# kallenordling/cesm_emulator

Measured on AMD Instinct MI355X. Metric: train samples/sec (192x288xT frames), higher is better.
Workload: dtype bf16; 1 GPU; config/more_blocks train step, F=12, 192x288, per-GPU batch 8; global_batch=8, frames=12, parallelism=dp1

## Files before the change

### cesm_emulator_amd/csrc/conv_wgrad.hip

```cpp
#include "conv_common.h"

namespace {

constexpr int WG_BP = 32;

template <typename T>
__global__ __launch_bounds__(256) void conv_wgrad_kernel(const T* __restrict__ x1, const T* __restrict__ x2,
                                                         const T* __restrict__ dy1, const T* __restrict__ dy2,
                                                         float* __restrict__ slab, ConvGeom g, int64_t M,
                                                         int64_t px_per_split) {
  constexpr int VEC = sizeof(T) == 2 ? 8 : 4;
  constexpr int ROW = 64;
  constexpr int LDR = sizeof(T) == 2 ? 64 : 65;
  __shared__ __attribute__((aligned(16))) T tY[2][WG_BP * LDR];
  __shared__ __attribute__((aligned(16))) T tX[2][WG_BP * LDR];

  const int tid = threadIdx.x, lane = tid & 63, wid = tid >> 6;
  const int wr = wid >> 1, wc = wid & 1;
  const int Cin = g.C1 + g.C2;
  const int co0 = blockIdx.x * 64;
  const int kcol0 = blockIdx.y * 64;
  const int tap = kcol0 / Cin;
  const int ci0 = kcol0 - tap * Cin;
  const int ky = tap / g.KW, kx = tap - ky * g.KW;
// ... 264 lines not shown
    for (int j = 0; j < 4; ++j) {
#pragma unroll
      for (int half = 0; half < 2; ++half) {
        const int r = lg * 8 + half * 4 + q;
        const int ch = ((j * 16 >> 2) + pp) ^ wgb_swz<64>(r);
        const s16x4 v = __builtin_amdgcn_ds_read_tr16_b64_v4i16((LDS_PTR(s16x4))(tX[buf] + r * 64 + ch * 4));
#pragma unroll
        for (int e = 0; e < 4; ++e) bfr[j][half * 4 + e] = __builtin_bit_cast(bf16, (short)v[e]);
      }
    }
#pragma unroll
    for (int i = 0; i < MT; ++i)
#pragma unroll
      for (int j = 0; j < 4; ++j) acc[i][j] = __builtin_amdgcn_mfma_f32_16x16x32_bf16(af[i], bfr[j], acc[i][j], 0, 0, 0);
    if constexpr (BIAS) {
      if (bias_blk) {
#pragma unroll
        for (int i = 0; i < MT; ++i) bacc[i] = __builtin_amdgcn_mfma_f32_16x16x32_bf16(af[i], ones, bacc[i], 0, 0, 0);
      }
    }
    if (s + 1 < nsteps) sstore(std::integral_constant<int, buf ^ 1>{});
    __syncthreads();
  };
  for (int s = 0; s < nsteps; s += 2) {
    step(s, I0{});
    if (s + 1 < nsteps) step(s + 1, I1{});
  }
  if (BIAS && bias_blk && lr == 0) {
#pragma unroll
    for (int i = 0; i < (BIAS ? MT : 1); ++i)
#pragma unroll
      for (int r = 0; r < 4; ++r) bslab[(int64_t)bz * g.Cout + co0 + wid * (BM / 4) + i * 16 + lg * 4 + r] = bacc[i][r];
  }
  const int K = g.KH * g.KW * Cin;
  float* out = slab + (int64_t)bz * g.Cout * K;
#pragma unroll
  for (int i = 0; i < MT; ++i)
#pragma unroll
    for (int j = 0; j < 4; ++j) {
      const int kc = kcol0 + j * 16 + lr;
#pragma unroll
      for (int r = 0; r < 4; ++r) {
        const int co = co0 + wid * (BM / 4) + i * 16 + lg * 4 + r;
        out[(int64_t)co * K + kc] = acc[i][j][r];
      }
    }
}

template <int BM, int BN, bool BIAS = false>
__global__ __launch_bounds__(512) __attribute__((amdgpu_waves_per_eu(2))) void wgrad_sq_kernel(
    const bf16* __restrict__ x, const bf16* __restrict__ dy, float* __restrict__ slab, float* __restrict__ bslab, int M,
    int Cout, int Cin, int px_per_split) {
  constexpr int WR = BM / 64, WC = 8 / WR, MT = 4, NT = BN / (16 * WC);
  static_assert((BM == 256 || BM == 64) && NT >= 1, "wgrad_sq tiles");
  constexpr int TY = WG_BP * BM / 8, TX = WG_BP * BN / 8;
  constexpr int NY = (TY + 511) / 512, NX = (TX + 511) / 512;
  __shared__ __attribute__((aligned(16))) bf16 tY[2][WG_BP * BM];
  __shared__ __attribute__((aligned(16))) bf16 tX[2][WG_BP * BN];
  const int tid = threadIdx.x, lane = tid & 63, wid = tid >> 6;
  const int lr = lane & 15, lg = lane >> 4;
  const int wr = wid % WR, wc = wid / WR;
  const int co0 = blockIdx.x * BM, k0 = blockIdx.y * BN;
  const int pbeg = blockIdx.z * px_per_split;
  const int pend = min(M, pbeg + px_per_split);
  bf16x8 yr2[2][NY], xr2[2][NX];
  auto gload = [&](int p0, auto slotc) {
    constexpr int slot = decltype(slotc)::value;
#pragma unroll
    for (int u = 0; u < NY; ++u) {
      const int v = tid + 512 * u, r = v / (BM / 8), c = (v % (BM / 8)) * 8;
      const int m = p0 + r;
      yr2[slot][u] = m < pend && v < TY ? *reinterpret_cast<const bf16x8*>(dy + (int64_t)m * Cout + co0 + c) : bf16x8{};
    }
#pragma unroll
    for (int u = 0; u < NX; ++u) {
      const int v = tid + 512 * u, r = v / (BN / 8), c = (v % (BN / 8)) * 8;
      const int m = p0 + r;
      xr2[slot][u] = m < pend && v < TX ? *reinterpret_cast<const bf16x8*>(x + (int64_t)m * Cin + k0 + c) : bf16x8{};
    }
  };
  auto sstore = [&](auto bufc) {
    constexpr int buf = decltype(bufc)::value;
#pragma unroll
    for (int u = 0; u < NY; ++u) {
      const int v = tid + 512 * u, r = v / (BM / 8), c = (v % (BM / 8)) * 8;
      if (v < TY) *reinterpret_cast<bf16x8*>(tY[buf] + r * BM + (((c >> 2) ^ wgb_swz<BM>(r)) * 4)) = yr2[buf][u];
    }
#pragma unroll
    for (int u = 0; u < NX; ++u) {
      const int v = tid + 512 * u, r = v / (BN / 8), c = (v % (BN / 8)) * 8;
      if (v < TX) *reinterpret_cast<bf16x8*>(tX[buf] + r * BN + (((c >> 2) ^ wgb_swz<BN>(r)) * 4)) = xr2[buf][u];
    }
  };
  f32x4 acc[MT][NT];
#pragma unroll
  for (int i = 0; i < MT; ++i)
#pragma unroll
    for (int j = 0; j < NT; ++j) acc[i][j] = f32x4{0.f, 0.f, 0.f, 0.f};
  const bool bias_w = BIAS && blockIdx.y == 0 && wc == 0;
  f32x4 bacc[BIAS ? MT : 1];
#pragma unroll
  for (int i = 0; i < (BIAS ? MT : 1); ++i) bacc[i] = f32x4{0.f, 0.f, 0.f, 0.f};
  bf16x8 ones;
#pragma unroll
  for (int e = 0; e < 8; ++e) ones[e] = (bf16)1.f;
  const int nsteps = (pend - pbeg + WG_BP - 1) / WG_BP;
  using I0 = std::integral_constant<int, 0>;
  using I1 = std::integral_constant<int, 1>;
  if (nsteps > 0) {
    gload(pbeg, I0{});
    if (nsteps > 1) gload(pbeg + WG_BP, I1{});
    sstore(I0{});
  }
  __syncthreads();
  const int q = lr >> 2, pp = lr & 3;
  auto step = [&](int s, auto bufc) {
    constexpr int buf = decltype(bufc)::value;
    if (s + 2 < nsteps) gload(pbeg + (s + 2) * WG_BP, bufc);
    bf16x8 af[MT], bfr[NT];
#pragma unroll
    for (int i = 0; i < MT; ++i) {
      const int c0 = wr * 64 + i * 16;
#pragma unroll
      for (int half = 0; half < 2; ++half) {
        const int r = lg * 8 + half * 4 + q;
        const int ch = ((c0 >> 2) + pp) ^ wgb_swz<BM>(r);
        const s16x4 v = __builtin_amdgcn_ds_read_tr16_b64_v4i16((LDS_PTR(s16x4))(tY[buf] + r * BM + ch * 4));
#pragma unroll
        for (int e = 0; e < 4; ++e) af[i][half * 4 + e] = __builtin_bit_cast(bf16, (short)v[e]);
      }
    }
#pragma unroll
    for (int j = 0; j < NT; ++j) {
      const int c0 = wc * (BN / WC) + j * 16;
#pragma unroll
      for (int half = 0; half < 2; ++half) {
        const int r = lg * 8 + half * 4 + q;
        const int ch = ((c0 >> 2) + pp) ^ wgb_swz<BN>(r);
        const s16x4 v = __builtin_amdgcn_ds_read_tr16_b64_v4i16((LDS_PTR(s16x4))(tX[buf] + r * BN + ch * 4));
#pragma unroll
        for (int e = 0; e < 4; ++e) bfr[j][half * 4 + e] = __builtin_bit_cast(bf16, (short)v[e]);
      }
    }
#pragma unroll
    for (int i = 0; i < MT; ++i)
#pragma unroll
      for (int j = 0; j < NT; ++j) acc[i][j] = __builtin_amdgcn_mfma_f32_16x16x32_bf16(af[i], bfr[j], acc[i][j], 0, 0, 0);
    if constexpr (BIAS) {
      if (bias_w) {
#pragma unroll
        for (int i = 0; i < MT; ++i) bacc[i] = __builtin_amdgcn_mfma_f32_16x16x32_bf16(af[i], ones, bacc[i], 0, 0, 0);
      }
    }
    if (s + 1 < nsteps) sstore(std::integral_constant<int, buf ^ 1>{});
    __syncthreads();
  };
  for (int s = 0; s < nsteps; s += 2) {
    step(s, I0{});
    if (s + 1 < nsteps) step(s + 1, I1{});
  }
  if (BIAS && bias_w && lr == 0) {
#pragma unroll
    for (int i = 0; i < (BIAS ? MT : 1); ++i)
#pragma unroll
      for (int r = 0; r < 4; ++r) bslab[(int64_t)blockIdx.z * Cout + co0 + wr * 64 + i * 16 + lg * 4 + r] = bacc[i][r];
  }
  float* out = slab + (int64_t)blockIdx.z * Cout * Cin;
#pragma unroll
  for (int i = 0; i < MT; ++i)
#pragma unroll
    for (int j = 0; j < NT; ++j) {
      const int kc = k0 + wc * (BN / WC) + j * 16 + lr;
#pragma unroll
      for (int r = 0; r < 4; ++r) {
        const int co = co0 + wr * 64 + i * 16 + lg * 4 + r;
        out[(int64_t)co * Cin + kc] = acc[i][j][r];
      }
    }
}

constexpr int W3_TH = 8, W3_TW = 32;
constexpr int W3_HW = W3_TW + 2, W3_NPIX = (W3_TH + 2) * (W3_TW + 2);
constexpr int W3_P = 48;

__device__ __forceinline__ int w3_swz_dy(int r) { return (((r >> 1) & 1) << 2) | (((r >> 3) & 1) << 3); }
__device__ __forceinline__ int w3_swz_x(int r) { return ((r >> 3) & 1) << 2; }

constexpr int W3_PLANE = (W3_TH + 2) * W3_P * 32;

constexpr int WG_NT = 512;
constexpr int WG_NI = 2;
__global__ __launch_bounds__(WG_NT, 1) void wgrad3x3c64_kernel(const bf16* __restrict__ x1, const bf16* __restrict__ x2,
                                                             const bf16* __restrict__ dy1, const bf16* __restrict__ dy2,
                                                             float* __restrict__ slab, ConvGeom g, int tiles_x,
                                                             int ntiles) {
  __shared__ __attribute__((aligned(16))) bf16 sdy[W3_TH * W3_TW * 64];
  __shared__ __attribute__((aligned(16))) bf16 shx[2 * W3_PLANE];
  const int tid = threadIdx.x, lane = tid & 63, wid = tid >> 6;
  const int cot0 = (wid >> 2) * 2, cit = wid & 3;
  const int co0 = blockIdx.x * 64, ci0 = blockIdx.y * 64;
  const int Cin = g.C1 + g.C2;
  const bf16* xs; int xcs, xcc;
  if (ci0 < g.C1) { xs = x1; xcs = g.C1; xcc = ci0; } else { xs = x2; xcs = g.C2; xcc = ci0 - g.C1; }
  const bf16* ys; int ycs, ycc;
  const int Co2 = g.Cout - g.Co1;
  if (co0 < g.Co1) { ys = dy1; ycs = g.Co1; ycc = co0; } else { ys = dy2; ycs = Co2; ycc = co0 - g.Co1; }
  const int tiles_per_img = tiles_x * ((g.Ho + W3_TH - 1) / W3_TH);

  f32x4 acc[WG_NI][9];
#pragma unroll
  for (int i = 0; i < WG_NI; ++i)
#pragma unroll
    for (int t = 0; t < 9; ++t) acc[i][t] = f32x4{0.f, 0.f, 0.f, 0.f};

  const int lr = lane & 15, lg = lane >> 4, q = lr >> 2, pp = lr & 3;
  const bf16* shp = shx + (cit >> 1) * W3_PLANE;
  int aoff[WG_NI][2], boff[2][3];
#pragma unroll
  for (int half = 0; half < 2; ++half) {
    const int r = lg * 8 + half * 4 + q;
#pragma unroll
    for (int i = 0; i < WG_NI; ++i) aoff[i][half] = r * 64 + ((((cot0 + i) * 4 + pp) ^ w3_swz_dy(r)) * 4);
#pragma unroll
    for (int kx = 0; kx < 3; ++kx) boff[half][kx] = (r + kx) * 32 + ((((cit & 1) * 4 + pp) ^ w3_swz_x(r + kx)) * 4);
  }
  constexpr int YV = 2048 / WG_NT, HV = (W3_NPIX * 8 + WG_NT - 1) / WG_NT;
  bf16x8 yv[YV], hv[HV];
  auto gload = [&](int tile) {
    const int n = tile / tiles_per_img;
    const int rem = tile - n * tiles_per_img;
    const int ty = rem / tiles_x, tx = rem - ty * tiles_x;
    const int y0 = ty * W3_TH, x0 = tx * W3_TW;
#pragma unroll
    for (int k = 0; k < YV; ++k) {
      const int e = tid + k * WG_NT;
      const int p = e >> 3, part = e & 7;
      const int oy = y0 + (p >> 5), ox = x0 + (p & 31);
      const bool ok = oy < g.Ho && ox < g.Wo;
      const bf16x8 v = *reinterpret_cast<const bf16x8*>(
          ys + (ok ? (((int64_t)n * g.Ho + oy) * g.Wo + ox) * ycs : 0) + ycc + part * 8);
      yv[k] = ok ? v : bf16x8{};
    }
#pragma unroll
    for (int k = 0; k < HV; ++k) {
      const int e = tid + k * WG_NT;
      const int hp = e >> 3, part = e & 7;
      const int r = hp / W3_HW, c = hp - r * W3_HW;
      const int iy = y0 - 1 + r, ix = x0 - 1 + c;
      const bool ok = e < W3_NPIX * 8 && (unsigned)iy < (unsigned)g.Hi && (unsigned)ix < (unsigned)g.Wi;
      const bf16x8 v = *reinterpret_cast<const bf16x8*>(
          xs + (ok ? (((int64_t)n * g.Hi + iy) * g.Wi + ix) * xcs : 0) + xcc + part * 8);
      hv[k] = ok ? v : bf16x8{};
    }
  };
  __shared__ __attribute__((aligned(16))) int tdump[WG_NT];
  auto touch = [&](int tile) {
    const int n = tile / tiles_per_img;
    const int rem = tile - n * tiles_per_img;
    const int ty = rem / tiles_x, tx = rem - ty * tiles_x;
    const int y0 = ty * W3_TH, x0 = tx * W3_TW;
    const int64_t yimg = (int64_t)g.Ho * g.Wo * ycs, ximg = (int64_t)g.Hi * g.Wi * xcs;
    const __amdgpu_buffer_rsrc_t yrs =
        __builtin_amdgcn_make_buffer_rsrc((void*)(ys + n * yimg + ycc), (short)0, (int)(yimg * 2 - ycc * 2), 0x00020000);
    const __amdgpu_buffer_rsrc_t xrs =
        __builtin_amdgcn_make_buffer_rsrc((void*)(xs + n * ximg + xcc), (short)0, (int)(ximg * 2 - xcc * 2), 0x00020000);
    auto* dst = (__attribute__((address_space(3))) void*)(tdump + wid * 64);
    {
      const int p = tid & 255;
      const int oy = y0 + (p >> 5), ox = x0 + (p & 31);
      const bool ok = tid < 256 && oy < g.Ho && ox < g.Wo;
      __builtin_amdgcn_raw_ptr_buffer_load_lds(yrs, dst, 4, ok ? (oy * g.Wo + ox) * ycs * 2 : 0x7ffffff0, 0, 0, 0);
    }
    {
      const int hp = tid < 256 ? 256 + tid : tid - 256;
      const int r = hp / W3_HW, c = hp - r * W3_HW;
      const int iy = y0 - 1 + r, ix = x0 - 1 + c;
      const bool ok = hp < W3_NPIX && (unsigned)iy < (unsigned)g.Hi && (unsigned)ix < (unsigned)g.Wi;
      __builtin_amdgcn_raw_ptr_buffer_load_lds(xrs, dst, 4, ok ? (iy * g.Wi + ix) * xcs * 2 : 0x7ffffff0, 0, 0, 0);
    }
  };
  if ((int)blockIdx.z < ntiles) gload(blockIdx.z);
  for (int tile = blockIdx.z; tile < ntiles; tile += gridDim.z) {
    __syncthreads();
#pragma unroll
    for (int k = 0; k < YV; ++k) {
      const int e = tid + k * WG_NT;
      const int p = e >> 3, part = e & 7;
      const int ch = (part * 2) ^ w3_swz_dy(p);
      *reinterpret_cast<bf16x8*>(sdy + p * 64 + ch * 4) = yv[k];
    }
#pragma unroll
    for (int k = 0; k < HV; ++k) {
      const int e = tid + k * WG_NT;
      if (e < W3_NPIX * 8) {
        const int hp = e >> 3, part = e & 7;
        const int r = hp / W3_HW, row = r * W3_P + (hp - r * W3_HW);
        const int ch = ((part & 3) * 2) ^ w3_swz_x(row);
        *reinterpret_cast<bf16x8*>(shx + (part >> 2) * W3_PLANE + row * 32 + ch * 4) = hv[k];
      }
    }
    __syncthreads();
    if (tile + (int)gridDim.z < ntiles) gload(tile + gridDim.z);
    if (tile + 2 * (int)gridDim.z < ntiles) touch(tile + 2 * gridDim.z);
    bf16x8 fa[2][WG_NI], fb[2][9];
    auto rd = [&](int py, int b) {
#pragma unroll
      for (int i = 0; i < WG_NI; ++i)
#pragma unroll
        for (int half = 0; half < 2; ++half) {
          const s16x4 v = __builtin_amdgcn_ds_read_tr16_b64_v4i16((LDS_PTR(s16x4))(sdy + aoff[i][half] + py * 32 * 64));
#pragma unroll
          for (int e = 0; e < 4; ++e) fa[b][i][half * 4 + e] = __builtin_bit_cast(bf16, (short)v[e]);
        }
#pragma unroll
      for (int tap = 0; tap < 9; ++tap) {
        const int ky = tap / 3, kx = tap - ky * 3;
#pragma unroll
        for (int half = 0; half < 2; ++half) {
          const s16x4 v = __builtin_amdgcn_ds_read_tr16_b64_v4i16(
              (LDS_PTR(s16x4))(shp + boff[half][kx] + (py + ky) * W3_P * 32));
#pragma unroll
          for (int e = 0; e < 4; ++e) fb[b][tap][half * 4 + e] = __builtin_bit_cast(bf16, (short)v[e]);
        }
      }
    };
    auto mm = [&](int b) {
#pragma unroll
      for (int tap = 0; tap < 9; ++tap)
#pragma unroll
        for (int i = 0; i < WG_NI; ++i)
          acc[i][tap] = __builtin_amdgcn_mfma_f32_16x16x32_bf16(fa[b][i], fb[b][tap], acc[i][tap], 0, 0, 0);
    };
    rd(0, 0);
#pragma unroll
    for (int py = 0; py < W3_TH; ++py) {
      const int b = py & 1;
      __builtin_amdgcn_sched_barrier(0);
      if (py + 1 < W3_TH) rd(py + 1, b ^ 1);
      mm(b);
      if (py + 1 < W3_TH) {
        constexpr int NRD = 2 * WG_NI + 18, NMF = 9 * WG_NI;
        constexpr int NPAIR = NRD < NMF ? NRD : NMF;
#pragma unroll
        for (int q2 = 0; q2 < NPAIR; ++q2) {
          __builtin_amdgcn_sched_group_barrier(0x100, 1, 0);
          __builtin_amdgcn_sched_group_barrier(0x008, 1, 0);
        }
        if (NRD > NPAIR) __builtin_amdgcn_sched_group_barrier(0x100, NRD - NPAIR, 0);
        if (NMF > NPAIR) __builtin_amdgcn_sched_group_barrier(0x008, NMF - NPAIR, 0);
      }
      __builtin_amdgcn_sched_barrier(0);
    }
  }
  const int K = 9 * Cin;
  float* out = slab + (int64_t)blockIdx.z * g.Cout * K;
#pragma unroll
  for (int i = 0; i < WG_NI; ++i)
#pragma unroll
    for (int tap = 0; tap < 9; ++tap) {
      const int ci = ci0 + cit * 16 + lr;
#pragma unroll
      for (int r = 0; r < 4; ++r) {
        const int co = co0 + (cot0 + i) * 16 + lg * 4 + r;
        out[(int64_t)co * K + tap * Cin + ci] = acc[i][tap][r];
      }
    }
}

template <int BY, int BX>
__device__ __forceinline__ void ws2_taps(const bf16* sdy, const bf16* shx, const int (&aoff)[2][2],
                                         const int (&boff)[2][3], f32x4 (&acc)[2][4]) {
#pragma unroll 1
  for (int py = 0; py < W3_TH; ++py) {
    bf16x8 af[2];
#pragma unroll
    for (int i = 0; i < 2; ++i) {
#pragma unroll
      for (int half = 0; half < 2; ++half) {
        const s16x4 v = __builtin_amdgcn_ds_read_tr16_b64_v4i16((LDS_PTR(s16x4))(sdy + aoff[i][half] + py * 32 * 64));
#pragma unroll
        for (int e = 0; e < 4; ++e) af[i][half * 4 + e] = __builtin_bit_cast(bf16, (short)v[e]);
      }
    }
#pragma unroll
    for (int t = 0; t < 4; ++t) {
      const int oy = BY + (t >> 1), ox = BX + (t & 1);
      bf16x8 bfr;
#pragma unroll
      for (int half = 0; half < 2; ++half) {
        const s16x4 v =
            __builtin_amdgcn_ds_read_tr16_b64_v4i16((LDS_PTR(s16x4))(shx + boff[half][ox] + (py + oy) * W3_P * 32));
#pragma unroll
        for (int e = 0; e < 4; ++e) bfr[half * 4 + e] = __builtin_bit_cast(bf16, (short)v[e]);
      }
      acc[0][t] = __builtin_amdgcn_mfma_f32_16x16x32_bf16(af[0], bfr, acc[0][t], 0, 0, 0);
      acc[1][t] = __builtin_amdgcn_mfma_f32_16x16x32_bf16(af[1], bfr, acc[1][t], 0, 0, 0);
    }
  }
}

__global__ __launch_bounds__(256, 2) void wgrads2_bf16_kernel(const bf16* __restrict__ x, const bf16* __restrict__ dy,
                                                              float* __restrict__ slab, ConvGeom g, int tiles_x,
                                                              int ntiles) {
  __shared__ __attribute__((aligned(16))) bf16 sdy[W3_TH * W3_TW * 64];
  __shared__ __attribute__((aligned(16))) bf16 shx[(W3_TH + 2) * W3_P * 32];
  const int tid = threadIdx.x, lane = tid & 63, wid = tid >> 6;
  const int cot0 = (wid >> 1) * 2, cit = wid & 1;
  const int co0 = blockIdx.x * 64;
  const int ab = (int)blockIdx.y & 3, a = ab >> 1, b = ab & 1;
  const int ci0 = ((int)blockIdx.y >> 2) * 32;
  const int Cin = g.C1;
  const int tiles_per_img = tiles_x * ((g.Ho + W3_TH - 1) / W3_TH);

  f32x4 acc[2][4];
#pragma unroll
  for (int i = 0; i < 2; ++i)
#pragma unroll
    for (int t = 0; t < 4; ++t) acc[i][t] = f32x4{0.f, 0.f, 0.f, 0.f};

  const int lr = lane & 15, lg = lane >> 4, q = lr >> 2, pp = lr & 3;
  int aoff[2][2], boff[2][3];
#pragma unroll
  for (int half = 0; half < 2; ++half) {
    const int r = lg * 8 + half * 4 + q;
#pragma unroll
    for (int i = 0; i < 2; ++i) aoff[i][half] = r * 64 + ((((cot0 + i) * 4 + pp) ^ w3_swz_dy(r)) * 4);
#pragma unroll
    for (int kx = 0; kx < 3; ++kx) boff[half][kx] = (r + kx) * 32 + (((cit * 4 + pp) ^ w3_swz_x(r + kx)) * 4);
  }
  for (int tile = blockIdx.z; tile < ntiles; tile += gridDim.z) {
    const int n = tile / tiles_per_img;
    const int rem = tile - n * tiles_per_img;
    const int ty = rem / tiles_x, tx = rem - ty * tiles_x;
    const int y0 = ty * W3_TH, x0 = tx * W3_TW;
    __syncthreads();
    {
      bf16x8 yv[8], hv[6];
#pragma unroll
      for (int k = 0; k < 8; ++k) {
        const int e = tid + k * 256;
        const int p = e >> 3, part = e & 7;
        const int oy = y0 + (p >> 5), ox = x0 + (p & 31);
        bf16x8 v = {};
        if (oy < g.Ho && ox < g.Wo)
          v = *reinterpret_cast<const bf16x8*>(dy + (((int64_t)n * g.Ho + oy) * g.Wo + ox) * g.Cout + co0 + part * 8);
        yv[k] = v;
      }
#pragma unroll
      for (int k = 0; k < 6; ++k) {
        const int e = tid + k * 256;
        bf16x8 v = {};
        if (e < W3_NPIX * 4) {
          const int hp = e >> 2, part = e & 3;
          const int r = hp / W3_HW, c = hp - r * W3_HW;
          const int iy = 2 * (y0 - 1 + r) + a, ix = 2 * (x0 - 1 + c) + b;
          if ((unsigned)iy < (unsigned)g.Hi && (unsigned)ix < (unsigned)g.Wi)
            v = *reinterpret_cast<const bf16x8*>(x + (((int64_t)n * g.Hi + iy) * g.Wi + ix) * Cin + ci0 + part * 8);
        }
        hv[k] = v;
      }
#pragma unroll
      for (int k = 0; k < 8; ++k) {
        const int e = tid + k * 256;
        const int p = e >> 3, part = e & 7;
        const int ch = (part * 2) ^ w3_swz_dy(p);
        *reinterpret_cast<bf16x8*>(sdy + p * 64 + ch * 4) = yv[k];
      }
#pragma unroll
      for (int k = 0; k < 6; ++k) {
        const int e = tid + k * 256;
        if (e < W3_NPIX * 4) {
          const int hp = e >> 2, part = e & 3;
          const int r = hp / W3_HW, row = r * W3_P + (hp - r * W3_HW);
          const int ch = (part * 2) ^ w3_swz_x(row);
          *reinterpret_cast<bf16x8*>(shx + row * 32 + ch * 4) = hv[k];
        }
      }
    }
    __syncthreads();
    switch (ab) {
      case 0: ws2_taps<1, 1>(sdy, shx, aoff, boff, acc); break;
      case 1: ws2_taps<1, 0>(sdy, shx, aoff, boff, acc); break;
      case 2: ws2_taps<0, 1>(sdy, shx, aoff, boff, acc); break;
      default: ws2_taps<0, 0>(sdy, shx, aoff, boff, acc); break;
    }
  }
  const int K = 16 * Cin;
  float* out = slab + (int64_t)blockIdx.z * g.Cout * K;
#pragma unroll
  for (int i = 0; i < 2; ++i)
#pragma unroll
    for (int t = 0; t < 4; ++t) {
      const int tap = (1 - a + 2 * (t >> 1)) * 4 + (1 - b + 2 * (t & 1));
      const int ci = ci0 + cit * 16 + lr;
#pragma unroll
      for (int r = 0; r < 4; ++r) {
        const int co = co0 + (cot0 + i) * 16 + lg * 4 + r;
        out[(int64_t)co * K + tap * Cin + ci] = acc[i][t][r];
      }
    }
}

constexpr int W36_TH = 8, W36_TW = 36, W36_HW = W36_TW + 2, W36_NPIX = (W36_TH + 2) * W36_HW;
constexpr int W36_NP = W36_TH * W36_TW;

__global__ __launch_bounds__(WG_NT, 1) void wgrad3x3w36c64_kernel(const bf16* __restrict__ x1, const bf16* __restrict__ x2,
                                                                const bf16* __restrict__ dy1, const bf16* __restrict__ dy2,
                                                                float* __restrict__ slab, ConvGeom g, int tiles_x,
                                                                int ntiles) {
  __shared__ __attribute__((aligned(16))) bf16 sdy[W36_NP * 64];
  __shared__ __attribute__((aligned(16))) bf16 shx[2 * W3_PLANE];
  const int tid = threadIdx.x, lane = tid & 63, wid = tid >> 6;
  const int cot0 = (wid >> 2) * 2, cit = wid & 3;
  const int co0 = blockIdx.x * 64, ci0 = blockIdx.y * 64;
  const int Cin = g.C1 + g.C2;
  const bf16* xs; int xcs, xcc;
  if (ci0 < g.C1) { xs = x1; xcs = g.C1; xcc = ci0; } else { xs = x2; xcs = g.C2; xcc = ci0 - g.C1; }
  const bf16* ys; int ycs, ycc;
  const int Co2 = g.Cout - g.Co1;
  if (co0 < g.Co1) { ys = dy1; ycs = g.Co1; ycc = co0; } else { ys = dy2; ycs = Co2; ycc = co0 - g.Co1; }
  const int tiles_per_img = tiles_x * ((g.Ho + W36_TH - 1) / W36_TH);

  f32x4 acc[WG_NI][9];
#pragma unroll
  for (int i = 0; i < WG_NI; ++i)
#pragma unroll
    for (int t = 0; t < 9; ++t) acc[i][t] = f32x4{0.f, 0.f, 0.f, 0.f};

  const int lr = lane & 15, lg = lane >> 4, q = lr >> 2, pp = lr & 3;
  const bf16* shp = shx + (cit >> 1) * W3_PLANE;
  const int cx = (cit & 1) * 4 + pp;
  int aoff[WG_NI][2];
#pragma unroll
  for (int half = 0; half < 2; ++half) {
    const int r = lg * 8 + half * 4 + q;
#pragma unroll
    for (int i = 0; i < WG_NI; ++i) aoff[i][half] = r * 64 + ((((cot0 + i) * 4 + pp) ^ w3_swz_dy(r)) * 4);
  }
  constexpr int YV = (W36_NP * 8 + WG_NT - 1) / WG_NT, HV = (W36_NPIX * 8 + WG_NT - 1) / WG_NT;
  bf16x8 yv[YV], hv[HV];
  auto gload = [&](int tile) {
    const int n = tile / tiles_per_img;
    const int rem = tile - n * tiles_per_img;
    const int ty = rem / tiles_x, tx = rem - ty * tiles_x;
    const int y0 = ty * W36_TH, x0 = tx * W36_TW;
#pragma unroll
    for (int k = 0; k < YV; ++k) {
      const int e = tid + k * WG_NT;
      const int p = e >> 3, part = e & 7;
      const int oy = y0 + p / W36_TW, ox = x0 + (p - (p / W36_TW) * W36_TW);
      const bool ok = e < W36_NP * 8 && oy < g.Ho && ox < g.Wo;
      const bf16x8 v = *reinterpret_cast<const bf16x8*>(
          ys + (ok ? (((int64_t)n * g.Ho + oy) * g.Wo + ox) * ycs : 0) + ycc + part * 8);
      yv[k] = ok ? v : bf16x8{};
    }
#pragma unroll
    for (int k = 0; k < HV; ++k) {
      const int e = tid + k * WG_NT;
      const int hp = e >> 3, part = e & 7;
      const int r = hp / W36_HW, c = hp - r * W36_HW;
      const int iy = y0 - 1 + r, ix = x0 - 1 + c;
      const bool ok = e < W36_NPIX * 8 && (unsigned)iy < (unsigned)g.Hi && (unsigned)ix < (unsigned)g.Wi;
      const bf16x8 v = *reinterpret_cast<const bf16x8*>(
          xs + (ok ? (((int64_t)n * g.Hi + iy) * g.Wi + ix) * xcs : 0) + xcc + part * 8);
      hv[k] = ok ? v : bf16x8{};
    }
  };
  if ((int)blockIdx.z < ntiles) gload(blockIdx.z);
  for (int tile = blockIdx.z; tile < ntiles; tile += gridDim.z) {
    __syncthreads();
#pragma unroll
    for (int k = 0; k < YV; ++k) {
      const int e = tid + k * WG_NT;
      if (e < W36_NP * 8) {
        const int p = e >> 3, part = e & 7;
        const int ch = (part * 2) ^ w3_swz_dy(p);
        *reinterpret_cast<bf16x8*>(sdy + p * 64 + ch * 4) = yv[k];
      }
    }
#pragma unroll
    for (int k = 0; k < HV; ++k) {
      const int e = tid + k * WG_NT;
      if (e < W36_NPIX * 8) {
        const int hp = e >> 3, part = e & 7;
        const int r = hp / W36_HW, row = r * W3_P + (hp - r * W36_HW);
        const int ch = ((part & 3) * 2) ^ w3_swz_x(row);
        *reinterpret_cast<bf16x8*>(shx + (part >> 2) * W3_PLANE + row * 32 + ch * 4) = hv[k];
      }
    }
    __syncthreads();
    if (tile + (int)gridDim.z < ntiles) gload(tile + gridDim.z);
    int prow[2], pcol[2];
#pragma unroll
    for (int half = 0; half < 2; ++half) { prow[half] = 0; pcol[half] = lg * 8 + half * 4 + q; }
    bf16x8 fa[2][WG_NI], fb[2][9];
    auto rd = [&](int kc, int b) {
#pragma unroll
      for (int i = 0; i < WG_NI; ++i)
#pragma unroll
        for (int half = 0; half < 2; ++half) {
          const s16x4 v = __builtin_amdgcn_ds_read_tr16_b64_v4i16((LDS_PTR(s16x4))(sdy + aoff[i][half] + kc * 32 * 64));
#pragma unroll
          for (int e = 0; e < 4; ++e) fa[b][i][half * 4 + e] = __builtin_bit_cast(bf16, (short)v[e]);
        }
      int bo[2][3];
#pragma unroll
      for (int half = 0; half < 2; ++half) {
        const int hb = prow[half] * W3_P + pcol[half];
#pragma unroll
        for (int kx = 0; kx < 3; ++kx) bo[half][kx] = (hb + kx) * 32 + ((cx ^ w3_swz_x(hb + kx)) * 4);
        pcol[half] += 32;
        if (pcol[half] >= W36_TW) { pcol[half] -= W36_TW; ++prow[half]; }
      }
#pragma unroll
      for (int tap = 0; tap < 9; ++tap) {
        const int ky = tap / 3, kx = tap - ky * 3;
#pragma unroll
        for (int half = 0; half < 2; ++half) {
          const s16x4 v = __builtin_amdgcn_ds_read_tr16_b64_v4i16((LDS_PTR(s16x4))(shp + bo[half][kx] + ky * W3_P * 32));
#pragma unroll
          for (int e = 0; e < 4; ++e) fb[b][tap][half * 4 + e] = __builtin_bit_cast(bf16, (short)v[e]);
        }
      }
    };
    auto mm = [&](int b) {
#pragma unroll
      for (int tap = 0; tap < 9; ++tap) {
#pragma unroll
        for (int i = 0; i < WG_NI; ++i)
          acc[i][tap] = __builtin_amdgcn_mfma_f32_16x16x32_bf16(fa[b][i], fb[b][tap], acc[i][tap], 0, 0, 0);
      }
    };
    constexpr int NKC = W36_NP / 32;
    rd(0, 0);
#pragma unroll
    for (int kc = 0; kc < NKC; ++kc) {
      const int b = kc & 1;
      __builtin_amdgcn_sched_barrier(0);
      if (kc + 1 < NKC) rd(kc + 1, b ^ 1);
      mm(b);
      if (kc + 1 < NKC) {
        constexpr int NRD = 2 * WG_NI + 18, NMF = 9 * WG_NI;
        constexpr int NPAIR = NRD < NMF ? NRD : NMF;
#pragma unroll
        for (int q2 = 0; q2 < NPAIR; ++q2) {
          __builtin_amdgcn_sched_group_barrier(0x100, 1, 0);
          __builtin_amdgcn_sched_group_barrier(0x008, 1, 0);
        }
        if (NRD > NPAIR) __builtin_amdgcn_sched_group_barrier(0x100, NRD - NPAIR, 0);
        if (NMF > NPAIR) __builtin_amdgcn_sched_group_barrier(0x008, NMF - NPAIR, 0);
      }
      __builtin_amdgcn_sched_barrier(0);
    }
  }
  const int K = 9 * Cin;
  float* out = slab + (int64_t)blockIdx.z * g.Cout * K;
#pragma unroll
  for (int i = 0; i < WG_NI; ++i)
#pragma unroll
    for (int tap = 0; tap < 9; ++tap) {
      const int ci = ci0 + cit * 16 + lr;
#pragma unroll
      for (int r = 0; r < 4; ++r) {
        const int co = co0 + (cot0 + i) * 16 + lg * 4 + r;
        out[(int64_t)co * K + tap * Cin + ci] = acc[i][tap][r];
      }
    }
}

__global__ __launch_bounds__(256) void conv_wgrad_reduce_kernel(const float* __restrict__ slab, float* __restrict__ dst,
                                                                int nsplit, int Cout, int Cin, int KH, int KW, int swap,
                                                                int flip, int accumulate) {
  const int64_t K = (int64_t)KH * KW * Cin;
  const int64_t total = (int64_t)Cout * K;
  const int64_t e = blockIdx.x * 64ll + (threadIdx.x & 63);
  const int grp = threadIdx.x >> 6;
  float s = 0.f;
  if (e < total) {
    int k = grp;
    for (; k + 28 < nsplit; k += 32) {
      float v[8];
#pragma unroll
      for (int u = 0; u < 8; ++u) v[u] = slab[(int64_t)(k + 4 * u) * total + e];
#pragma unroll
      for (int u = 0; u < 8; ++u) s += v[u];
    }
    for (; k < nsplit; k += 4) s += slab[(int64_t)k * total + e];
  }
  __shared__ float red[4][64];
  red[grp][threadIdx.x & 63] = s;
  __syncthreads();
  if (grp != 0 || e >= total) return;
  s = ((red[0][threadIdx.x] + red[1][threadIdx.x]) + red[2][threadIdx.x]) + red[3][threadIdx.x];
  const int co = (int)(e / K);
  const int kc = (int)(e - (int64_t)co * K);
  const int tap = kc / Cin, ci = kc - tap * Cin;
  int ky = tap / KW, kx = tap - ky * KW;
  if (flip) { ky = KH - 1 - ky; kx = KW - 1 - kx; }
  const int d0 = swap ? ci : co, d1 = swap ? co : ci, D1 = swap ? Cout : Cin;
  const int64_t di = (((int64_t)d0 * D1 + d1) * KH + ky) * KW + kx;
  dst[di] = accumulate ? dst[di] + s : s;
}

template <typename T>
__global__ void colsum_partial_kernel(const T* __restrict__ x, float* __restrict__ part, int64_t rows, int C,
                                      int64_t rows_per_split) {
  const int cq = C / 4;
  const int rl = 256 / cq;
  const int tid = threadIdx.x;
  const int q = tid % cq, rr = tid / cq;
  __shared__ float red[256 * 4];
  float s[4] = {0.f, 0.f, 0.f, 0.f};
  const int64_t r0 = blockIdx.x * rows_per_split;
  const int64_t r1 = min(rows, r0 + rows_per_split);
  if (rr < rl) {
    for (int64_t r = r0 + rr; r < r1; r += rl) {
      float v[4];
      load4(x + r * C + q * 4, v);
      s[0] += v[0]; s[1] += v[1]; s[2] += v[2]; s[3] += v[3];
    }
  }
  for (int i = 0; i < 4; ++i) red[tid * 4 + i] = s[i];
  __syncthreads();
  if (tid < cq) {
    float t[4] = {0.f, 0.f, 0.f, 0.f};
    for (int k = 0; k < rl; ++k)
      for (int i = 0; i < 4; ++i) t[i] += red[(k * cq + tid) * 4 + i];
    for (int i = 0; i < 4; ++i) part[(int64_t)blockIdx.x * C + tid * 4 + i] = t[i];
  }
}

__global__ void colsum_final_kernel(const float* __restrict__ part, float* __restrict__ dst, int nsplit, int C,
                                    int accumulate) {
  const int c = blockIdx.x;
  float s = 0.f;
  for (int k = threadIdx.x; k < nsplit; k += 64) s += part[(int64_t)k * C + c];
  s = wave_sum(s);
  if (threadIdx.x == 0) dst[c] = accumulate ? dst[c] + s : s;
}

enum WgradVariant { WGV_WIDE = 0, WGV_SQ, WGV_GEN, WGV_S2, WGV_W32C64, WGV_W36C64 };

constexpr int WG_BLOCKS = 1024;
constexpr int WG_BLOCKS_BIG = 512;
constexpr int WG_BLOCKS_SQ = 256;
constexpr int WG_BLOCKS_SQ64 = 512;
constexpr int WG_SPLIT_PX = 256;

struct WgradPlan {
  WgradVariant v = WGV_GEN;
  int bm = 64, bn = 64;
  int nsplit = 1;
  bool bias = false;
  bool can_bias = false;
};

static WgradPlan wgrad_plan(int dtype, int Nb, int Hi, int Wi, int C1, int C2, int Ho, int Wo, int Cout, int Co1,
                            int KH, int KW, int S, int P, int U, bool with_bias) {
  WgradPlan pl;
  const bool bf = dtype == CESM_DT_BF16;
  const int Cin = C1 + C2, K = KH * KW * Cin;
  const int64_t M = (int64_t)Nb * Ho * Wo;
  const bool same_hw = Ho == Hi && Wo == Wi, single = C2 == 0 && Co1 == Cout;
  int64_t blocks = WG_BLOCKS, tiles;
  if (bf && KH == 3 && KW == 3 && S == 1 && P == 1 && U == 1 && same_hw) {
    pl.v = ((Wo % W36_TW) == 0 && 5 * Wo <= 4 * (int)cdiv(Wo, W3_TW) * W3_TW) ? WGV_W36C64 : WGV_W32C64;
    blocks = WG_BLOCKS_BIG;
    tiles = (int64_t)(Cout / 64) * (Cin / 32);
  } else if (bf && KH == 4 && KW == 4 && S == 2 && P == 1 && U == 1 && Hi == 2 * Ho && Wi == 2 * Wo && Wo >= 64 &&
             single && !with_bias) {
    pl.v = WGV_S2;
    blocks = WG_BLOCKS_BIG;
    tiles = (int64_t)(Cout / 64) * (Cin / 32) * 4;
  } else {
    const bool wide = bf && M < (1ll << 31);
    int sq = 0;
    if (wide && KH == 1 && KW == 1 && S == 1 && P == 0 && U == 1 && same_hw && single) {
      if (Cout == 64) sq = C1 % 256 == 0 ? 256 : 0;
      else if (Cout % 256 == 0) sq = C1 % 256 == 0 ? 256 : (C1 % 128 == 0 ? 128 : 0);
    }
    pl.v = sq ? WGV_SQ : (wide ? WGV_WIDE : WGV_GEN);
    if (sq) {
      pl.bm = Cout == 64 ? 64 : 256;
      pl.bn = sq;
      blocks = pl.bm == 64 ? WG_BLOCKS_SQ64 : WG_BLOCKS_SQ;
    } else {
      pl.bm = !bf ? 64 : (Cout % 256 == 0 && Co1 % 256 == 0) ? 256 : (Cout % 128 == 0 && Co1 % 128 == 0) ? 128 : 64;
      blocks = pl.bm == 256 ? WG_BLOCKS_BIG : WG_BLOCKS;
    }
    tiles = (int64_t)std::max(1, Cout / pl.bm) * std::max(1, K / pl.bn);
    pl.bias = with_bias && wide;
    pl.can_bias = wide && Co1 == Cout;
  }
  pl.nsplit = (int)std::max<int64_t>(
      1, std::min(blocks / std::max<int64_t>(1, tiles), std::max<int64_t>(1, M / WG_SPLIT_PX)));
  return pl;
}
}

extern "C" {

const char* cesm_conv_wgrad_variant(int dtype, int Nb, int Hi, int Wi, int C1, int C2, int Ho, int Wo, int Cout,
                                    int Co1, int KH, int KW, int S, int P, int U, int with_bias) {
  const WgradPlan pl = wgrad_plan(dtype, Nb, Hi, Wi, C1, C2, Ho, Wo, Cout, Co1, KH, KW, S, P, U, with_bias != 0);
  switch (pl.v) {
    case WGV_W32C64: return "wgrad3x3c64_kernel";
    case WGV_W36C64: return "wgrad3x3w36c64_kernel";
    case WGV_S2: return "wgrads2_bf16_kernel";
    case WGV_SQ: {
      static const char* const sqn[6] = {"wgrad_sq_kernel<64,256>", "wgrad_sq_kernel<64,256,true>",
                                         "wgrad_sq_kernel<256,256>", "wgrad_sq_kernel<256,256,true>",
                                         "wgrad_sq_kernel<256,128>", "wgrad_sq_kernel<256,128,true>"};
      return sqn[(pl.bm == 64 ? 0 : pl.bn == 256 ? 2 : 4) + (with_bias ? 1 : 0)];
    }
    case WGV_WIDE: {
      static const char* const names[6] = {"wgrad_wide_kernel<64,false>", "wgrad_wide_kernel<64,true>",
                                           "wgrad_wide_kernel<128,false>", "wgrad_wide_kernel<128,true>",
                                           "wgrad_wide_kernel<256,false>", "wgrad_wide_kernel<256,true>"};
      return names[(pl.bm == 256 ? 4 : pl.bm == 128 ? 2 : 0) + (with_bias ? 1 : 0)];
    }
    default: return dtype == CESM_DT_BF16 ? "conv_wgrad_kernel<__bf16>" : "conv_wgrad_kernel<float>";
  }
}

int cesm_conv_wgrad_nsplit(int dtype, int Nb, int Hi, int Wi, int C1, int C2, int Ho, int Wo, int Cout, int Co1, int KH,
                           int KW, int S, int P, int U, int with_bias) {
  return wgrad_plan(dtype, Nb, Hi, Wi, C1, C2, Ho, Wo, Cout, Co1, KH, KW, S, P, U, with_bias != 0).nsplit;
}

int cesm_conv_wgrad_bias_rides(int dtype, int Nb, int Hi, int Wi, int C1, int C2, int Ho, int Wo, int Cout, int Co1,
                               int KH, int KW, int S, int P, int U) {
  return wgrad_plan(dtype, Nb, Hi, Wi, C1, C2, Ho, Wo, Cout, Co1, KH, KW, S, P, U, false).can_bias ? 1 : 0;
}

int cesm_conv_wgrad(int dtype, const void* x1, const void* x2, const void* dy1, const void* dy2, float* dw,
                    float* slab, float* db, float* bslab, int nsplit, int Nb, int Hi, int Wi, int C1, int C2, int Ho,
                    int Wo, int Cout, int Co1, int KH, int KW, int S, int P, int U, int swap, int flip, int accumulate,
                    hipStream_t stream) {
  if (db && !bslab) return CESM_EINVAL;
  const int Cin = C1 + C2;
  if ((Cin % 64) || (C1 % 64) || (Cout % 64) || (Co1 % 64) || nsplit <= 0) return CESM_EINVAL;
  if (dtype != CESM_DT_BF16 && dtype != CESM_DT_F32) return CESM_EINVAL;
  const WgradPlan pl = wgrad_plan(dtype, Nb, Hi, Wi, C1, C2, Ho, Wo, Cout, Co1, KH, KW, S, P, U, db != nullptr);
  if (db && !pl.bias) return CESM_EUNSUPPORTED;
  ConvGeom g{Nb, Hi, Wi, Ho, Wo, C1, C2, Cout, Co1, KH, KW, S, P, U};
  const int64_t M = (int64_t)Nb * Ho * Wo;
  const int64_t pps = cdiv(cdiv(M, nsplit), WG_BP) * WG_BP;
  const int K = KH * KW * Cin;
  switch (pl.v) {
    case WGV_W36C64: {
      const int tx = Wo / W36_TW;
      const int ntiles = Nb * tx * (int)cdiv(Ho, W36_TH);
      dim3 g3(Cout / 64, Cin / 64, std::min(nsplit, ntiles));
      wgrad3x3w36c64_kernel<<<g3, WG_NT, 0, stream>>>((const bf16*)x1, (const bf16*)x2, (const bf16*)dy1,
                                                    (const bf16*)dy2, slab, g, tx, ntiles);
      nsplit = (int)g3.z;
      break;
    }
    case WGV_W32C64: {
      const int tx = (int)cdiv(Wo, W3_TW);
      const int ntiles = Nb * tx * (int)cdiv(Ho, W3_TH);
      dim3 g3(Cout / 64, Cin / 64, std::min(nsplit, ntiles));
      wgrad3x3c64_kernel<<<g3, WG_NT, 0, stream>>>((const bf16*)x1, (const bf16*)x2, (const bf16*)dy1,
                                                 (const bf16*)dy2, slab, g, tx, ntiles);
      nsplit = (int)g3.z;
      break;
    }
    case WGV_S2: {
      const int tx = (int)cdiv(Wo, W3_TW);
      const int ntiles = Nb * tx * (int)cdiv(Ho, W3_TH);
      dim3 g3(Cout / 64, (Cin / 32) * 4, std::min(nsplit, ntiles));
      wgrads2_bf16_kernel<<<g3, 256, 0, stream>>>((const bf16*)x1, (const bf16*)dy1, slab, g, tx, ntiles);
      nsplit = (int)g3.z;
      break;
    }
    case WGV_SQ: {
      const dim3 gq(Cout / pl.bm, Cin / pl.bn, nsplit);
      const bf16 *qx = (const bf16*)x1, *qy = (const bf16*)dy1;
#define SQL(BMv, BNv, Bv) \
  wgrad_sq_kernel<BMv, BNv, Bv><<<gq, 512, 0, stream>>>(qx, qy, slab, bslab, (int)M, Cout, Cin, (int)pps)
      if (pl.bm == 64) { if (db) SQL(64, 256, true); else SQL(64, 256, false); }
      else if (pl.bn == 256) { if (db) SQL(256, 256, true); else SQL(256, 256, false); }
      else { if (db) SQL(256, 128, true); else SQL(256, 128, false); }
#undef SQL
      break;
    }
    case WGV_WIDE: {
      const dim3 gw(Cout / pl.bm, K / 64, nsplit);
      auto launch = [&](auto bmc, auto biasc) {
        constexpr int BMv = decltype(bmc)::value;
        constexpr bool Bv = decltype(biasc)::value;
        wgrad_wide_kernel<BMv, Bv><<<gw, 256, 0, stream>>>((const bf16*)x1, (const bf16*)x2, (const bf16*)dy1,
                                                           (const bf16*)dy2, slab, bslab, g, (int)M, (int)pps);
      };
      using T0 = std::false_type;
      using T1 = std::true_type;
      if (pl.bm == 256) { if (db) launch(std::integral_constant<int, 256>{}, T1{}); else launch(std::integral_constant<int, 256>{}, T0{}); }
      else if (pl.bm == 128) { if (db) launch(std::integral_constant<int, 128>{}, T1{}); else launch(std::integral_constant<int, 128>{}, T0{}); }
      else { if (db) launch(std::integral_constant<int, 64>{}, T1{}); else launch(std::integral_constant<int, 64>{}, T0{}); }
      break;
    }
    case WGV_GEN: {
      dim3 grid(Cout / 64, K / 64, nsplit);
      if (dtype == CESM_DT_BF16)
        conv_wgrad_kernel<bf16><<<grid, 256, 0, stream>>>((const bf16*)x1, (const bf16*)x2, (const bf16*)dy1,
                                                          (const bf16*)dy2, slab, g, M, pps);
      else
        conv_wgrad_kernel<float><<<grid, 256, 0, stream>>>((const float*)x1, (const float*)x2, (const float*)dy1,
                                                           (const float*)dy2, slab, g, M, pps);
      break;
    }
  }
  if (db) colsum_final_kernel<<<Cout, 64, 0, stream>>>(bslab, db, nsplit, Cout, 1);
  const int64_t total = (int64_t)Cout * K;
  conv_wgrad_reduce_kernel<<<(unsigned)cdiv(total, 64), 256, 0, stream>>>(slab, dw, nsplit, Cout, Cin, KH, KW, swap,
                                                                          flip, accumulate);
  return cesm_launch_status();
}

int cesm_colsum(int dtype, const void* x, float* dst, float* part, int nsplit, int64_t rows, int C, int accumulate,
                hipStream_t stream) {
  if (C % 4 || C > 1024 || nsplit <= 0) return CESM_EINVAL;
  const int64_t rps = cdiv(rows, nsplit);
  if (dtype == CESM_DT_BF16)
    colsum_partial_kernel<bf16><<<nsplit, 256, 0, stream>>>((const bf16*)x, part, rows, C, rps);
  else if (dtype == CESM_DT_F32)
    colsum_partial_kernel<float><<<nsplit, 256, 0, stream>>>((const float*)x, part, rows, C, rps);
  else
    return CESM_EINVAL;
  colsum_final_kernel<<<C, 64, 0, stream>>>(part, dst, nsplit, C, accumulate);
  return cesm_launch_status();
}

}
```

Baseline: 64.35 samples/s.

## Reuse halo-row B fragments across kernel rows in 3x3 wgrad kernels

Restructures the wgrad inner loops so the LDS-read B fragments of each halo row are kept in a rolling register buffer and shared across the three ky taps. Each output row then needs only one new halo row per step instead of rereading all nine taps. The change applies to the main 3x3 kernel, the stride-2 tap helper and the W36 variant, where the W36 tail is handled by a separate prologue. This cuts LDS read traffic and rebalances the read/MFMA interleave schedule, at the cost of more live VGPRs and more intricate indexing, which could affect occupancy or correctness.

Result: no change. 64.80 samples/s, median of 6 (+0.7%).

```diff
diff --git a/cesm_emulator_amd/csrc/conv_wgrad.hip b/cesm_emulator_amd/csrc/conv_wgrad.hip
--- a/cesm_emulator_amd/csrc/conv_wgrad.hip
+++ b/cesm_emulator_amd/csrc/conv_wgrad.hip
@@ -590,52 +590,61 @@
     __syncthreads();
     if (tile + (int)gridDim.z < ntiles) gload(tile + gridDim.z);
     if (tile + 2 * (int)gridDim.z < ntiles) touch(tile + 2 * gridDim.z);
-    bf16x8 fa[2][WG_NI], fb[2][9];
-    auto rd = [&](int py, int b) {
+    bf16x8 fa[2][WG_NI], hb[4][3];
+    auto rda = [&](int py) {
 #pragma unroll
       for (int i = 0; i < WG_NI; ++i)
 #pragma unroll
         for (int half = 0; half < 2; ++half) {
           const s16x4 v = __builtin_amdgcn_ds_read_tr16_b64_v4i16((LDS_PTR(s16x4))(sdy + aoff[i][half] + py * 32 * 64));
 #pragma unroll
-          for (int e = 0; e < 4; ++e) fa[b][i][half * 4 + e] = __builtin_bit_cast(bf16, (short)v[e]);
-        }
-#pragma unroll
-      for (int tap = 0; tap < 9; ++tap) {
-        const int ky = tap / 3, kx = tap - ky * 3;
+          for (int e = 0; e < 4; ++e) fa[py & 1][i][half * 4 + e] = __builtin_bit_cast(bf16, (short)v[e]);
+        }
+    };
+    auto rdb = [&](int hr) {
+#pragma unroll
+      for (int kx = 0; kx < 3; ++kx)
 #pragma unroll
         for (int half = 0; half < 2; ++half) {
-          const s16x4 v = __builtin_amdgcn_ds_read_tr16_b64_v4i16(
-              (LDS_PTR(s16x4))(shp + boff[half][kx] + (py + ky) * W3_P * 32));
-#pragma unroll
-          for (int e = 0; e < 4; ++e) fb[b][tap][half * 4 + e] = __builtin_bit_cast(bf16, (short)v[e]);
-        }
-      }
+          const s16x4 v =
+              __builtin_amdgcn_ds_read_tr16_b64_v4i16((LDS_PTR(s16x4))(shp + boff[half][kx] + hr * W3_P * 32));
+#pragma unroll
+          for (int e = 0; e < 4; ++e) hb[hr & 3][kx][half * 4 + e] = __builtin_bit_cast(bf16, (short)v[e]);
+        }
     };
-    auto mm = [&](int b) {
+    auto mm = [&](int py) {
 #pragma unroll
       for (int tap = 0; tap < 9; ++tap)
 #pragma unroll
         for (int i = 0; i < WG_NI; ++i)
-          acc[i][tap] = __builtin_amdgcn_mfma_f32_16x16x32_bf16(fa[b][i], fb[b][tap], acc[i][tap], 0, 0, 0);
+          acc[i][tap] = __builtin_amdgcn_mfma_f32_16x16x32_bf16(fa[py & 1][i], hb[(py + tap / 3) & 3][tap % 3],
+                                                                acc[i][tap], 0, 0, 0);
     };
-    rd(0, 0);
+    rda(0);
+    rdb(0);
+    rdb(1);
+    rdb(2);
 #pragma unroll
     for (int py = 0; py < W3_TH; ++py) {
-      const int b = py & 1;
       __builtin_amdgcn_sched_barrier(0);
-      if (py + 1 < W3_TH) rd(py + 1, b ^ 1);
-      mm(b);
       if (py + 1 < W3_TH) {
-        constexpr int NRD = 2 * WG_NI + 18, NMF = 9 * WG_NI;
-        constexpr int NPAIR = NRD < NMF ? NRD : NMF;
-#pragma unroll
-        for (int q2 = 0; q2 < NPAIR; ++q2) {
+        rdb(py + 3);
+        rda(py + 1);
+      }
+      mm(py);
+      if (py + 1 < W3_TH) {
+        constexpr int NRD = 2 * WG_NI + 6, NMF = 9 * WG_NI;
+        static_assert(NRD <= NMF && NMF <= 2 * NRD, "1 read : 1 or 2 MFMAs");
+#pragma unroll
+        for (int q2 = 0; q2 < NMF - NRD; ++q2) {
+          __builtin_amdgcn_sched_group_barrier(0x100, 1, 0);
+          __builtin_amdgcn_sched_group_barrier(0x008, 2, 0);
+        }
+#pragma unroll
+        for (int q2 = 0; q2 < 2 * NRD - NMF; ++q2) {
           __builtin_amdgcn_sched_group_barrier(0x100, 1, 0);
           __builtin_amdgcn_sched_group_barrier(0x008, 1, 0);
         }
-        if (NRD > NPAIR) __builtin_amdgcn_sched_group_barrier(0x100, NRD - NPAIR, 0);
-        if (NMF > NPAIR) __builtin_amdgcn_sched_group_barrier(0x008, NMF - NPAIR, 0);
       }
       __builtin_amdgcn_sched_barrier(0);
     }
@@ -658,31 +667,42 @@
 template <int BY, int BX>
 __device__ __forceinline__ void ws2_taps(const bf16* sdy, const bf16* shx, const int (&aoff)[2][2],
                                          const int (&boff)[2][3], f32x4 (&acc)[2][4]) {
-#pragma unroll 1
-  for (int py = 0; py < W3_TH; ++py) {
-    bf16x8 af[2];
-#pragma unroll
-    for (int i = 0; i < 2; ++i) {
-#pragma unroll
-      for (int half = 0; half < 2; ++half) {
-        const s16x4 v = __builtin_amdgcn_ds_read_tr16_b64_v4i16((LDS_PTR(s16x4))(sdy + aoff[i][half] + py * 32 * 64));
-#pragma unroll
-        for (int e = 0; e < 4; ++e) af[i][half * 4 + e] = __builtin_bit_cast(bf16, (short)v[e]);
-      }
-    }
-#pragma unroll
-    for (int t = 0; t < 4; ++t) {
-      const int oy = BY + (t >> 1), ox = BX + (t & 1);
-      bf16x8 bfr;
+  auto rdb = [&](bf16x8 (&dst)[2], int hr) {
+#pragma unroll
+    for (int u = 0; u < 2; ++u)
 #pragma unroll
       for (int half = 0; half < 2; ++half) {
         const s16x4 v =
-            __builtin_amdgcn_ds_read_tr16_b64_v4i16((LDS_PTR(s16x4))(shx + boff[half][ox] + (py + oy) * W3_P * 32));
-#pragma unroll
-        for (int e = 0; e < 4; ++e) bfr[half * 4 + e] = __builtin_bit_cast(bf16, (short)v[e]);
-      }
-      acc[0][t] = __builtin_amdgcn_mfma_f32_16x16x32_bf16(af[0], bfr, acc[0][t], 0, 0, 0);
-      acc[1][t] = __builtin_amdgcn_mfma_f32_16x16x32_bf16(af[1], bfr, acc[1][t], 0, 0, 0);
+            __builtin_amdgcn_ds_read_tr16_b64_v4i16((LDS_PTR(s16x4))(shx + boff[half][BX + u] + hr * W3_P * 32));
+#pragma unroll
+        for (int e = 0; e < 4; ++e) dst[u][half * 4 + e] = __builtin_bit_cast(bf16, (short)v[e]);
+      }
+  };
+  bf16x8 rows[2][2];
+  rdb(rows[0], BY);
+  static_assert(W3_TH % 2 == 0, "the row loop advances by two");
+#pragma unroll 1
+  for (int py0 = 0; py0 < W3_TH; py0 += 2) {
+#pragma unroll
+    for (int s = 0; s < 2; ++s) {
+      const int py = py0 + s;
+      bf16x8 af[2];
+#pragma unroll
+      for (int i = 0; i < 2; ++i) {
+#pragma unroll
+        for (int half = 0; half < 2; ++half) {
+          const s16x4 v = __builtin_amdgcn_ds_read_tr16_b64_v4i16((LDS_PTR(s16x4))(sdy + aoff[i][half] + py * 32 * 64));
+#pragma unroll
+          for (int e = 0; e < 4; ++e) af[i][half * 4 + e] = __builtin_bit_cast(bf16, (short)v[e]);
+        }
+      }
+      rdb(rows[s ^ 1], py + BY + 1);
+#pragma unroll
+      for (int t = 0; t < 4; ++t) {
+        const bf16x8 bfr = rows[s ^ (t >> 1)][t & 1];
+        acc[0][t] = __builtin_amdgcn_mfma_f32_16x16x32_bf16(af[0], bfr, acc[0][t], 0, 0, 0);
+        acc[1][t] = __builtin_amdgcn_mfma_f32_16x16x32_bf16(af[1], bfr, acc[1][t], 0, 0, 0);
+      }
     }
   }
 }
@@ -818,12 +838,16 @@
   const int lr = lane & 15, lg = lane >> 4, q = lr >> 2, pp = lr & 3;
   const bf16* shp = shx + (cit >> 1) * W3_PLANE;
   const int cx = (cit & 1) * 4 + pp;
-  int aoff[WG_NI][2];
+  int aoff[2], atail[2], boff[2][3], btail[2];
 #pragma unroll
   for (int half = 0; half < 2; ++half) {
     const int r = lg * 8 + half * 4 + q;
-#pragma unroll
-    for (int i = 0; i < WG_NI; ++i) aoff[i][half] = r * 64 + ((((cot0 + i) * 4 + pp) ^ w3_swz_dy(r)) * 4);
+    aoff[half] = r * 64 + (((cot0 * 4 + pp) ^ w3_swz_dy(r)) * 4);
+    const int j = lg * 2 + half, pt = j * W36_TW + 32 + q;
+    atail[half] = pt * 64 + (((cot0 * 4 + pp) ^ w3_swz_dy(pt)) * 4);
+    btail[half] = (j * W3_P + 32 + q) * 32 + cx * 4;
+#pragma unroll
+    for (int kx = 0; kx < 3; ++kx) boff[half][kx] = (r + kx) * 32 + ((cx ^ w3_swz_x(r + kx)) * 4);
   }
   constexpr int YV = (W36_NP * 8 + WG_NT - 1) / WG_NT, HV = (W36_NPIX * 8 + WG_NT - 1) / WG_NT;
   bf16x8 yv[YV], hv[HV];
@@ -878,65 +902,78 @@
     }
     __syncthreads();
     if (tile + (int)gridDim.z < ntiles) gload(tile + gridDim.z);
-    int prow[2], pcol[2];
-#pragma unroll
-    for (int half = 0; half < 2; ++half) { prow[half] = 0; pcol[half] = lg * 8 + half * 4 + q; }
-    bf16x8 fa[2][WG_NI], fb[2][9];
-    auto rd = [&](int kc, int b) {
+    bf16x8 fa[2][WG_NI], ft[3][3], hb[4][3];
+    auto rda = [&](int slot, int off0, int off1, int row, int imm) {
 #pragma unroll
       for (int i = 0; i < WG_NI; ++i)
 #pragma unroll
         for (int half = 0; half < 2; ++half) {
-          const s16x4 v = __builtin_amdgcn_ds_read_tr16_b64_v4i16((LDS_PTR(s16x4))(sdy + aoff[i][half] + kc * 32 * 64));
-#pragma unroll
-          for (int e = 0; e < 4; ++e) fa[b][i][half * 4 + e] = __builtin_bit_cast(bf16, (short)v[e]);
-        }
-      int bo[2][3];
-#pragma unroll
-      for (int half = 0; half < 2; ++half) {
-        const int hb = prow[half] * W3_P + pcol[half];
-#pragma unroll
-        for (int kx = 0; kx < 3; ++kx) bo[half][kx] = (hb + kx) * 32 + ((cx ^ w3_swz_x(hb + kx)) * 4);
-        pcol[half] += 32;
-        if (pcol[half] >= W36_TW) { pcol[half] -= W36_TW; ++prow[half]; }
-      }
-#pragma unroll
-      for (int tap = 0; tap < 9; ++tap) {
-        const int ky = tap / 3, kx = tap - ky * 3;
+          const s16x4 v = __builtin_amdgcn_ds_read_tr16_b64_v4i16(
+              (LDS_PTR(s16x4))(sdy + ((half ? off1 : off0) ^ (i * 16 + (((half + row) >> 1) & 1) * 32)) + imm));
+#pragma unroll
+          for (int e = 0; e < 4; ++e) fa[slot][i][half * 4 + e] = __builtin_bit_cast(bf16, (short)v[e]);
+        }
+    };
+    auto rdrow = [&](int py) {
+      rda(py & 1, aoff[0], aoff[1], py, py * W36_TW * 64);
+    };
+    auto rdb = [&](bf16x8 (&dst)[3], int hr, bool tail) {
+#pragma unroll
+      for (int kx = 0; kx < 3; ++kx)
 #pragma unroll
         for (int half = 0; half < 2; ++half) {
-          const s16x4 v = __builtin_amdgcn_ds_read_tr16_b64_v4i16((LDS_PTR(s16x4))(shp + bo[half][kx] + ky * W3_P * 32));
-#pragma unroll
-          for (int e = 0; e < 4; ++e) fb[b][tap][half * 4 + e] = __builtin_bit_cast(bf16, (short)v[e]);
-        }
-      }
+          const int off = tail ? btail[half] + kx * 32 : boff[half][kx];
+          const s16x4 v = __builtin_amdgcn_ds_read_tr16_b64_v4i16((LDS_PTR(s16x4))(shp + off + hr * W3_P * 32));
+#pragma unroll
+          for (int e = 0; e < 4; ++e) dst[kx][half * 4 + e] = __builtin_bit_cast(bf16, (short)v[e]);
+        }
     };
-    auto mm = [&](int b) {
-#pragma unroll
-      for (int tap = 0; tap < 9; ++tap) {
+    rda(1, atail[0], atail[1], 0, 0);
+#pragma unroll
+    for (int ky = 0; ky < 3; ++ky) rdb(ft[ky], ky, true);
+    __builtin_amdgcn_sched_barrier(0);
+    rdb(hb[0], 0, false);
+    rdb(hb[1], 1, false);
+    rdb(hb[2], 2, false);
+    rdrow(0);
+#pragma unroll
+    for (int tap = 0; tap < 9; ++tap)
+#pragma unroll
+      for (int i = 0; i < WG_NI; ++i)
+        acc[i][tap] = __builtin_amdgcn_mfma_f32_16x16x32_bf16(fa[1][i], ft[tap / 3][tap % 3], acc[i][tap], 0, 0, 0);
+#pragma unroll
+    for (int q2 = 0; q2 < 9 * WG_NI; ++q2) {
+      __builtin_amdgcn_sched_group_barrier(0x100, 1, 0);
+      __builtin_amdgcn_sched_group_barrier(0x008, 1, 0);
+    }
+    __builtin_amdgcn_sched_group_barrier(0x100, 2 * WG_NI, 0);
+    __builtin_amdgcn_sched_barrier(0);
+#pragma unroll
+    for (int py = 0; py < W36_TH; ++py) {
+      __builtin_amdgcn_sched_barrier(0);
+      if (py + 1 < W36_TH) {
+        rdb(hb[(py + 3) & 3], py + 3, false);
+        rdrow(py + 1);
+      }
+#pragma unroll
+      for (int tap = 0; tap < 9; ++tap)
 #pragma unroll
         for (int i = 0; i < WG_NI; ++i)
-          acc[i][tap] = __builtin_amdgcn_mfma_f32_16x16x32_bf16(fa[b][i], fb[b][tap], acc[i][tap], 0, 0, 0);
-      }
-    };
-    constexpr int NKC = W36_NP / 32;
-    rd(0, 0);
-#pragma unroll
-    for (int kc = 0; kc < NKC; ++kc) {
-      const int b = kc & 1;
-      __builtin_amdgcn_sched_barrier(0);
-      if (kc + 1 < NKC) rd(kc + 1, b ^ 1);
-      mm(b);
-      if (kc + 1 < NKC) {
-        constexpr int NRD = 2 * WG_NI + 18, NMF = 9 * WG_NI;
-        constexpr int NPAIR = NRD < NMF ? NRD : NMF;
-#pragma unroll
-        for (int q2 = 0; q2 < NPAIR; ++q2) {
+          acc[i][tap] = __builtin_amdgcn_mfma_f32_16x16x32_bf16(fa[py & 1][i], hb[(py + tap / 3) & 3][tap % 3],
+                                                                acc[i][tap], 0, 0, 0);
+      if (py + 1 < W36_TH) {
+        constexpr int NRD = 2 * WG_NI + 6, NMF = 9 * WG_NI;
+        static_assert(NRD <= NMF && NMF <= 2 * NRD, "1 read : 1 or 2 MFMAs");
+#pragma unroll
+        for (int q2 = 0; q2 < NMF - NRD; ++q2) {
+          __builtin_amdgcn_sched_group_barrier(0x100, 1, 0);
+          __builtin_amdgcn_sched_group_barrier(0x008, 2, 0);
+        }
+#pragma unroll
+        for (int q2 = 0; q2 < 2 * NRD - NMF; ++q2) {
           __builtin_amdgcn_sched_group_barrier(0x100, 1, 0);
           __builtin_amdgcn_sched_group_barrier(0x008, 1, 0);
         }
-        if (NRD > NPAIR) __builtin_amdgcn_sched_group_barrier(0x100, NRD - NPAIR, 0);
-        if (NMF > NPAIR) __builtin_amdgcn_sched_group_barrier(0x008, NMF - NPAIR, 0);
       }
       __builtin_amdgcn_sched_barrier(0);
     }
```
